# marco-conciatori-public/weed_instance_segmentation

Hardware: AMD Instinct MI355X
Metric: images/sec at 1024x1024 bs=8 per GPU (Mask2Former R50, 100 queries, fp32 forward-only) (higher is better)
Workload: dtype f32

## Files before the change

include/wm2f.h:

```cpp
#ifndef WM2F_H
#define WM2F_H

#include <stdint.h>

#ifdef __cplusplus
extern "C" {
#endif

#define WM2F_VERSION 100

#define WM2F_F32 0
#define WM2F_BF16 1
#define WM2F_I32 2
#define WM2F_U8 3
#define WM2F_U16 4
#define WM2F_I64 5

#define WM2F_OK 0
#define WM2F_EINVAL (-1)
#define WM2F_EUNSUPPORTED (-2)
#define WM2F_ELAUNCH (-3)

#define WM2F_MAX_LEVELS 8

// ... 128 lines not shown
                                 const void* pos, void* y, void* y_bf16, void* y_plus_pos, int yp_dtype, void* stats,
                                 int64_t rows, int C, int64_t pos_rows, float eps, float clamp, void* stream);
int wm2f_add_layernorm_train_bwd(const void* x, int x_dtype, const void* residual, const void* gamma, const void* stats,
                                 const void* grad_y, const void* grad_y_bf16, const void* grad_y_plus_pos, int gyp_dtype,
                                 void* grad_sum, void* grad_x, void* grad_gamma, void* grad_beta, void* workspace,
                                 int64_t rows, int C, void* stream);
int wm2f_token_linear_fwd(const void* x, const void* w, const void* bias, const void* residual, const void* ln_gamma,
                          const void* ln_beta, const void* pos, void* out, void* out_plus_pos, int64_t M, int K, int N, int relu,
                          int64_t pos_rows, float eps, int out_group, void* stream);

int wm2f_token_linear_split_weight(const void* w, void* w_split, int N, int K, void* stream);
int wm2f_token_linear_split_fwd(const void* x, const void* w_split, const void* bias, const void* residual, const void* ln_gamma,
                                const void* ln_beta, const void* pos, void* out, void* out_plus_pos, int64_t M, int K, int N,
                                int relu, int64_t pos_rows, float eps, int out_group, void* stream);

int wm2f_conv1x1_split_fwd(const void* x, const void* w_split, const void* bias, const void* residual, void* out, int B, int K,
                           int N, int Hi, int Wi, int stride, int relu, int config, void* stream);
int wm2f_conv1x1_split_config(int N, int P, int B, int n_cu);

int wm2f_conv3x3_split_fwd(const void* x, const void* w_split, const void* bias, void* out, int B, int Cin, int N, int Hi,
                           int Wi, int stride, int relu, int config, void* stream);
int wm2f_conv3x3_split_config(int N, int P, int B, int n_cu);

int wm2f_conv1x1_split_gn_fwd(const void* x, const void* w_split, const void* bias, void* out, void* stats_out, int G_out,
                              const void* norm_stats, const void* norm_gamma, const void* norm_beta, int norm_G, float norm_eps,
                              int norm_relu, int B, int K, int N, int Hi, int Wi, int stride, int config, void* stream);
int wm2f_conv3x3_split_stats_fwd(const void* x, const void* w_split, void* out, void* stats_out, int G_out, int B, int Cin,
                                 int N, int Hi, int Wi, int stride, int config, void* stream);
int wm2f_group_norm_act_apply(const void* x, const void* gamma, const void* beta, const void* up, void* y, const void* stats,
                              int B, int C, int G, int H, int W, int Hs, int Ws, float eps, int relu, void* stream);
int wm2f_group_norm_tokens_apply(const void* x, const void* bias, const void* gamma, const void* beta, void* tokens,
                                 const void* stats, int B, int C, int G, int HW, int S, int start, float eps, void* stream);

int wm2f_stem7x7_pool_fwd(const void* x, const void* w_split, const void* bias, void* out, int B, int Cin, int N, int Hi,
                          int Wi, int grid, void* stream);

int wm2f_token_linear_split_fwd_p(const void* x, const void* w_split, const void* bias, const void* residual,
                                  const void* ln_gamma, const void* ln_beta, const void* pos, void* out, void* out_plus_pos,
                                  int64_t M, int K, int N, int relu, int64_t pos_rows, float eps, int out_group, int pieces,
                                  void* stream);
int wm2f_conv1x1_split_fwd_p(const void* x, const void* w_split, const void* bias, const void* residual, void* out, int B, int K,
                             int N, int Hi, int Wi, int stride, int relu, int config, int pieces, void* stream);
int wm2f_conv1x1_split_gn_fwd_p(const void* x, const void* w_split, const void* bias, void* out, void* stats_out, int G_out,
                                const void* norm_stats, const void* norm_gamma, const void* norm_beta, int norm_G, float norm_eps,
                                int norm_relu, int B, int K, int N, int Hi, int Wi, int stride, int config, int pieces,
                                void* stream);
int wm2f_conv3x3_split_fwd_p(const void* x, const void* w_split, const void* bias, void* out, int B, int Cin, int N, int Hi,
                             int Wi, int stride, int relu, int config, int pieces, void* stream);
int wm2f_conv3x3_split_stats_fwd_p(const void* x, const void* w_split, void* out, void* stats_out, int G_out, int B, int Cin,
                                   int N, int Hi, int Wi, int stride, int config, int pieces, void* stream);
int wm2f_stem7x7_pool_fwd_p(const void* x, const void* w_split, const void* bias, void* out, int B, int Cin, int N, int Hi,
                            int Wi, int grid, int pieces, void* stream);

int64_t wm2f_token_wgrad_workspace(int64_t M, int N, int K);
int wm2f_token_wgrad_bf16(const void* dy, const void* x, void* dw, void* db, void* workspace, int64_t M, int N, int K,
// ... 229 lines not shown
```

weed_instance_segmentation_amd/_lib.py:

```python
from __future__ import annotations

import ctypes
import os
from ctypes import POINTER, c_char_p, c_float, c_int, c_int32, c_int64, c_void_p

HERE = os.path.dirname(os.path.abspath(__file__))
LIB_PATH = os.path.join(HERE, "libwm2f.so")
PROF_LIB_PATH = os.path.join(HERE, "libwm2f_prof.so")
if os.environ.get("WM2F_PROF_LIB"):
    PROF_LIB_PATH = os.environ["WM2F_PROF_LIB"]

WM2F_F32 = 0
WM2F_BF16 = 1
WM2F_I32 = 2
WM2F_U8 = 3
WM2F_U16 = 4
WM2F_I64 = 5
WM2F_CCL_VALUE, WM2F_CCL_BINARY, WM2F_CCL_RGB = 0, 1, 2
WM2F_CCL_MAX_COLORS = 16
WM2F_POLY_MAX_SIDE = 16384
WM2F_POLY_MAX_COORD = 1 << 24
WM2F_RLE_MAX_IDS = 1024
WM2F_AUG_MAX_VIRTUAL = 65536
WM2F_TILE_MAX_SIDE, WM2F_TILE_MAX_IDS, WM2F_TILE_MAX_TILES, WM2F_TILE_MAX_PAIRS = 16384, 256, 1024, 16384
# ... 65 lines not shown
    "wm2f_matcher_workspace": (c_int64, [_I, _I, _I, _I, _I]),
    "wm2f_matcher_cost": (c_int, [_P, _P, _P, _I, _HOST_I32, _P, _P, _P, _P, _I, _I, _I, _I, _I, _I, _I, _I, _I, _I,
                                  c_float, c_float, c_float, _P]),
    "wm2f_matcher_cost_levels": (c_int, [POINTER(c_void_p), _P, _P, _I, _HOST_I32, _P, _P, _P, _P, _I, _I, _I, _I, _I, _I, _I,
                                         _I, _I, _I, c_float, c_float, c_float, _P]),
    "wm2f_lsa_batched": (c_int, [_P, _P, _P, _P, _I, _I, _I, _I, _I, _P]),
    "wm2f_add_broadcast": (c_int, [_P, _P, _P, _I, c_int64, _P]),
    "wm2f_bias_act": (c_int, [_P, _P, _P, _P, _I, _I, _I, _I, _P]),
    "wm2f_add_layernorm": (c_int, [_P, _P, _P, _P, _P, _P, _P, c_int64, _I, c_int64, c_float, _P]),
    "wm2f_add_layernorm_train_workspace": (c_int64, [c_int64]),
    "wm2f_add_layernorm_train_fwd": (c_int, [_P, _I, _P, _P, _P, _P, _P, _P, _P, _I, _P, c_int64, _I, c_int64, c_float, c_float, _P]),
    "wm2f_add_layernorm_train_bwd": (c_int, [_P, _I, _P, _P, _P, _P, _P, _P, _I, _P, _P, _P, _P, _P, c_int64, _I, _P]),
    "wm2f_token_linear_fwd": (c_int, [_P, _P, _P, _P, _P, _P, _P, _P, _P, c_int64, _I, _I, _I, c_int64, c_float, _I, _P]),
    "wm2f_token_linear_split_weight": (c_int, [_P, _P, _I, _I, _P]),
    "wm2f_token_linear_split_fwd": (c_int, [_P, _P, _P, _P, _P, _P, _P, _P, _P, c_int64, _I, _I, _I, c_int64, c_float, _I, _P]),
    "wm2f_conv1x1_split_config": (c_int, [_I, _I, _I, _I]),
    "wm2f_conv1x1_split_fwd": (c_int, [_P, _P, _P, _P, _P, _I, _I, _I, _I, _I, _I, _I, _I, _P]),
    "wm2f_conv3x3_split_config": (c_int, [_I, _I, _I, _I]),
    "wm2f_conv3x3_split_fwd": (c_int, [_P, _P, _P, _P, _I, _I, _I, _I, _I, _I, _I, _I, _P]),
    "wm2f_conv1x1_split_gn_fwd": (c_int, [_P, _P, _P, _P, _P, _I, _P, _P, _P, _I, c_float, _I, _I, _I, _I, _I, _I, _I, _I, _P]),
    "wm2f_conv3x3_split_stats_fwd": (c_int, [_P, _P, _P, _P, _I, _I, _I, _I, _I, _I, _I, _I, _P]),
    "wm2f_group_norm_act_apply": (c_int, [_P, _P, _P, _P, _P, _P, _I, _I, _I, _I, _I, _I, _I, c_float, _I, _P]),
    "wm2f_group_norm_tokens_apply": (c_int, [_P, _P, _P, _P, _P, _P, _I, _I, _I, _I, _I, _I, c_float, _P]),
    "wm2f_stem7x7_pool_fwd":(c_int, [_P, _P, _P, _P, _I, _I, _I, _I, _I, _I, _P]),
    "wm2f_token_linear_split_fwd_p": (c_int, [_P, _P, _P, _P, _P, _P, _P, _P, _P, c_int64, _I, _I, _I, c_int64, c_float, _I, _I, _P]),
    "wm2f_conv1x1_split_fwd_p": (c_int, [_P, _P, _P, _P, _P, _I, _I, _I, _I, _I, _I, _I, _I, _I, _P]),
    "wm2f_conv1x1_split_gn_fwd_p": (c_int, [_P, _P, _P, _P, _P, _I, _P, _P, _P, _I, c_float, _I, _I, _I, _I, _I, _I, _I, _I, _I, _P]),
    "wm2f_conv3x3_split_fwd_p": (c_int, [_P, _P, _P, _P, _I, _I, _I, _I, _I, _I, _I, _I, _I, _P]),
    "wm2f_conv3x3_split_stats_fwd_p": (c_int, [_P, _P, _P, _P, _I, _I, _I, _I, _I, _I, _I, _I, _I, _P]),
    "wm2f_stem7x7_pool_fwd_p": (c_int, [_P, _P, _P, _P, _I, _I, _I, _I, _I, _I, _I, _P]),
    "wm2f_token_wgrad_workspace": (c_int64, [c_int64, _I, _I]),
    "wm2f_token_wgrad_bf16": (c_int, [_P, _P, _P, _P, _P, c_int64, _I, _I, _P]),
    "wm2f_token_wgrad_f32": (c_int, [_P, _P, _P, _P, _P, c_int64, _I, _I, _P]),
    "wm2f_tokens_to_nchw": (c_int, [_P, _P, _I, _I, _I, _I, _I, _P]),
    "wm2f_group_norm_tokens": (c_int, [_P, _P, _P, _P, _P, _P, _I, _I, _I, _I, _I, _I, c_float, _P]),
    "wm2f_resize_bilinear": (c_int, [_P, _P, _I, _I, _I, _I, _I, _P]),
    "wm2f_resize_pyramid": (c_int, [_P, _P, _P, _P, _I, _I, _I, _P]),
    "wm2f_bias_relu_maxpool": (c_int, [_P, _P, _P, _I, _I, _I, _I, _P]),
    "wm2f_group_norm_act": (c_int, [_P, _P, _P, _P, _P, _P, _I, _I, _I, _I, _I, _I, _I, c_float, _I, _P]),
    "wm2f_point_sample_fwd": (c_int, [_P, _I, _P, _P, _P, _I, _I, _I, _I, _P]),
# ... 112 lines not shown
```

weed_instance_segmentation_amd/csrc/token_gemm_split.hip:

```cpp
#include "common.h"

namespace wm2f {
namespace {

using f32x4 = __attribute__((ext_vector_type(4))) float;
using f32x8 = __attribute__((ext_vector_type(8))) float;
using u32x4 = __attribute__((ext_vector_type(4))) unsigned int;
using bf16x8 = __attribute__((ext_vector_type(8))) __bf16;
typedef __attribute__((address_space(3))) void* lds_ptr_t;

constexpr int kSgWaves = 8;
constexpr int kSgThreads = kSgWaves * 64;
constexpr int kSgCT = 2;
constexpr int kKStep = 32;
constexpr int kFrag = 1024;
constexpr unsigned kOob = 0x80000000u;
constexpr float kBf16Max = 3.38953139e38f;

template <int P = 3>
__device__ __forceinline__ void split3(const f32x8 x, bf16x8& h, bf16x8& m, bf16x8& l) {
  f32x8 xc;
#pragma unroll
  for (int i = 0; i < 8; ++i) xc[i] = __builtin_amdgcn_fmed3f(x[i], -kBf16Max, kBf16Max);
  if constexpr (P == 1) {
// ... 5 lines not shown
    const f32x8 r1 = x - __builtin_convertvector(h, f32x8);
    m = __builtin_convertvector(r1, bf16x8);
    if constexpr (P >= 3) {
      const f32x8 r2 = r1 - __builtin_convertvector(m, f32x8);
      l = __builtin_convertvector(r2, bf16x8);
    }
  }
}

__global__ __launch_bounds__(256) void split_weight_kernel(const float* __restrict__ w, bf16x8* __restrict__ ws, int N, int K) {
  const int kg_n = K / 8;
  const int i = blockIdx.x * blockDim.x + threadIdx.x;
  if (i >= N * kg_n) return;
  const int n = i / kg_n, kg = i - n * kg_n;
  const f32x4* src = reinterpret_cast<const f32x4*>(w + (int64_t)n * K + kg * 8);
  const f32x4 lo = src[0], hi = src[1];
  const f32x8 v = {lo[0], lo[1], lo[2], lo[3], hi[0], hi[1], hi[2], hi[3]};
  bf16x8 h, m, l;
  split3(v, h, m, l);
  const int ks = kg >> 2, g = kg & 3, rt = n >> 4, lane = (n & 15) + 16 * g;
  const int64_t base = ((int64_t)ks * (N / 16) + rt) * 3 * 64 + lane;
  ws[base] = h;
  ws[base + 64] = m;
  ws[base + 128] = l;
}

struct SgArgs {
  const float *x, *bias, *residual, *gamma, *beta, *pos;
  const void* ws;
  float *out, *out_pos;
// ... 265 lines not shown
          } else {
#pragma unroll
            for (int rt = 0; rt < NRT; ++rt)
              __builtin_amdgcn_raw_buffer_store_b128(__builtin_bit_cast(u32x4, acc[rt][c]), o_rs, row_o + (unsigned)((rt * 16 + 4 * g) * 4), 0, 0);
          }
        }
#pragma unroll
        for (int rt = 0; rt < NRT; ++rt) acc[rt][c] = (f32x4){0.f, 0.f, 0.f, 0.f};
      }
    }
    if (q + 1 < n_q && late) issue(q + 1);
    sg_barrier();
  }
}

using sg_kernel_t = void (*)(SgArgs);

template <bool PIPE, int ABL, int P = 3>
sg_kernel_t sg_pick(bool n288, int epi) {
  if (n288) return epi == 2 ? token_gemm_split_kernel<18, 2, PIPE, ABL, P> : (epi == 1 ? token_gemm_split_kernel<18, 1, true, ABL, P> : token_gemm_split_kernel<18, 0, true, ABL, P>);
  return epi == 2 ? token_gemm_split_kernel<16, 2, PIPE, ABL, P> : (epi == 1 ? token_gemm_split_kernel<16, 1, true, ABL, P> : token_gemm_split_kernel<16, 0, true, ABL, P>);
}

int device_cu_count(int* n_cu) {
  static int cached = 0;
  if (cached == 0) {
    int dev = 0;
    hipDeviceProp_t prop;
    if (hipGetDevice(&dev) != hipSuccess || hipGetDeviceProperties(&prop, dev) != hipSuccess) return -1;
    cached = prop.multiProcessorCount;
// ... 5 lines not shown
}
}

using namespace wm2f;

extern "C" int wm2f_token_linear_split_weight(const void* w, void* w_split, int N, int K, void* stream) {
  const char* who = "wm2f_token_linear_split_weight";
  WM2F_REQUIRE(w && w_split, "%s: null pointer", who);
  WM2F_REQUIRE(N > 0 && K > 0 && N % 16 == 0 && K % kKStep == 0, "%s: N = %d must be a multiple of 16 and K = %d of %d", who, N, K, kKStep);
  WM2F_REQUIRE((int64_t)N * K * 6 < (1ll << 31), "%s: the split weight must stay below 2 GiB", who);
  const int total = N * (K / 8);
  hipLaunchKernelGGL(split_weight_kernel, dim3((total + 255) / 256), dim3(256), 0, (hipStream_t)stream, (const float*)w,
                     (bf16x8*)w_split, N, K);
  WM2F_CHECK_LAUNCH(who);
  return WM2F_OK;
}

static int token_split_launch(const char* who, const void* x, const void* w_split, const void* bias, const void* residual,
                              const void* ln_gamma, const void* ln_beta, const void* pos, void* out, void* out_plus_pos,
                              int64_t M, int K, int N, int relu, int64_t pos_rows, float eps, int out_group, int pieces,
                              void* stream) {
  WM2F_REQUIRE(pieces >= 1 && pieces <= 3, "%s: pieces = %d (1, 2 and 3 are built)", who, pieces);
  WM2F_REQUIRE(x && w_split && bias && out, "%s: null pointer", who);
  WM2F_REQUIRE(M > 0 && K > 0 && N > 0, "%s: non-positive size", who);
  WM2F_REQUIRE(N == 256 || N == 288 || N == 512 || N == 768 || N == 1024,
               "%s: N = %d is not built (256, 288 and multiples of 256 up to 1024 are)", who, N);
  WM2F_REQUIRE(K % kKStep == 0, "%s: K = %d must be a multiple of %d", who, K, kKStep);
  WM2F_REQUIRE(M * (int64_t)K * 4 < (1ll << 31) && M * (int64_t)N * 4 < (1ll << 31), "%s: x / out must stay below 2 GiB (32-bit buffer offsets)", who);
  WM2F_REQUIRE((int64_t)N * K * 6 < (1ll << 31), "%s: the split weight must stay below 2 GiB", who);
  WM2F_REQUIRE(pos_rows * (int64_t)N * 4 < (1ll << 31), "%s: pos must stay below 2 GiB", who);
// ... 79 lines not shown
```

weed_instance_segmentation_amd/modeling.py:

```python
from __future__ import annotations

import json
import math
import os
from typing import Sequence

import numpy as np
import torch
import torch.nn.functional as F
from torch import nn

from . import ops
from .backbone_resnet import build_backbone
from .configuration import Mask2FormerConfig
from .loss import Mask2FormerLoss


class Mask2FormerForUniversalSegmentationOutput:

    _fields = ("loss", "class_queries_logits", "masks_queries_logits", "auxiliary_logits", "encoder_last_hidden_state",
               "pixel_decoder_last_hidden_state", "transformer_decoder_last_hidden_state", "encoder_hidden_states",
               "pixel_decoder_hidden_states", "transformer_decoder_hidden_states", "attentions")

    def __init__(self, **kw):
# ... 124 lines not shown
        self.self_attn_layer_norm = nn.LayerNorm(d)
        self.dropout = config.dropout
        self.fc1 = nn.Linear(d, config.encoder_feedforward_dim)
        self.fc2 = nn.Linear(config.encoder_feedforward_dim, d)
        self.final_layer_norm = nn.LayerNorm(d)

    def forward(self, hidden, pos, ref, level_hw, hp=None, emit_next=True):
        hidden_lp = None
        if isinstance(hp, tuple):
            hp, hidden_lp = hp
        if (not torch.is_grad_enabled() and self.dropout == 0.0 and hidden.shape[-1] == 256
                and hidden.dtype == torch.float32 and not torch.is_autocast_enabled("cuda")):
            B_, S_, C_ = hidden.shape
            ln1, ln2 = self.self_attn_layer_norm, self.final_layer_norm
            op = self.self_attn.output_proj
            if (ops.token_linear_applies(hidden, op.weight) and ops.token_linear_applies(hidden, self.fc1.weight)
                    and B_ * S_ * self.fc1.out_features * 4 < (1 << 31)):
                a = self.self_attn(hidden, pos, ref, level_hw, hp, project=False)
                hidden = ops.token_linear(a, op.weight, op.bias, residual=hidden, ln=(ln1.weight, ln1.bias, ln1.eps),
                                          w_split=ops.split_weight_cached(self, "output_proj", op.weight))
                f = ops.token_linear(hidden, self.fc1.weight, self.fc1.bias, relu=True,
                                     w_split=ops.split_weight_cached(self, "fc1", self.fc1.weight))
                return ops.token_linear(f, self.fc2.weight, self.fc2.bias, residual=hidden, ln=(ln2.weight, ln2.bias, ln2.eps),
                                        pos=pos, w_split=ops.split_weight_cached(self, "fc2", self.fc2.weight))
            a = self.self_attn(hidden, pos, ref, level_hw, hp)
            hidden = ops.add_layernorm(a, hidden, ln1.weight, ln1.bias, ln1.eps)
            f = torch._addmm_activation(self.fc1.bias, hidden.reshape(B_ * S_, C_), self.fc1.weight.t(), use_gelu=False)
            f = self.fc2(f).view(B_, S_, C_)
            return ops.add_layernorm(f, hidden, ln2.weight, ln2.bias, ln2.eps, pos=pos)
        amp = torch.is_autocast_enabled("cuda")
        bf16 = amp and torch.get_autocast_dtype("cuda") == torch.bfloat16
        if (torch.is_grad_enabled() and self.dropout == 0.0 and hidden.is_cuda and hidden.shape[-1] == 256
                and hidden.dtype == torch.float32 and (bf16 or not amp)):
            ln1, ln2 = self.self_attn_layer_norm, self.final_layer_norm
            a = self.self_attn(hidden, pos, ref, level_hw, hp, hidden_lp)
# ... 596 lines not shown
```

weed_instance_segmentation_amd/ops/__init__.py:

```python
from __future__ import annotations

import os as _os

K1_BWD_DETERMINISTIC: bool | None = None

CONV1X1_SPLIT = True

CONV3X3_SPLIT = True

CONV_GN_FUSED = True

SPLIT_PRECISION: str | None = _os.environ.get("WM2F_SPLIT_PRECISION") or "highest"

from .._lib import check
from ._core import KernelTimer, _p, _stream, set_kernel_timer
from .ccl import label_components, resize_nearest_tables
from .clean import labelmap_clean
from .copy_paste import copy_paste
from .fused import (add_broadcast, bias_act_, bias_relu_maxpool, group_norm_act_, group_norm_act_from_stats_, group_norm_tokens_,
                    group_norm_tokens_from_stats_, resize_bilinear, resize_pyramid, tokens_to_nchw)
from .gemm import (conv1x1, conv1x1_applies, conv1x1_gn, conv3x3, conv3x3_applies, conv3x3_stats, conv_group_stats_applies,
                   linear_tokens, split_weight, split_weight_3x3,
                   split_weight_cached, split_weight_stem, stem_conv_pool, stem_conv_pool_applies, stem_weight_columns,
                   stem_weight_matrix, token_linear, token_linear_applies, token_wgrad, token_wgrad_applies)
from .k1 import (k1_bwd_deterministic, k1_lane_order, k1_lane_rows, k1_lanes_applies, k1_rows_applies, ms_deform_attn,
                 ms_deform_attn_bwd, ms_deform_attn_fused, ms_deform_attn_fused_lanes, ms_deform_attn_fused_packed,
                 ms_deform_attn_rows, ms_deform_attn_variant)
from .k2 import masked_xattn, masked_xattn_bf16_applies
from .k3 import (attn_mask_build, mask_einsum, mask_einsum_attn_mask, mask_einsum_bf16, mask_einsum_bf16_bwd,
                 mask_einsum_bf16_bwd_applies, mask_einsum_bwd, mask_einsum_bwd_applies, nchw_to_pixel_major_bf16)
from .labelmaps import (coco_match, coco_match_min, labelmap_aim_points, labelmap_boundary, labelmap_distance,
                        labelmap_instance_stats, labelmap_pair_counts, labelmap_to_masks, mask_pair_counts, panoptic_match,
                        semantic_confusion_)
from .layernorm import add_layernorm, add_layernorm_train, add_layernorm_train_applies
from .loss import mask_loss_rows, point_sample, point_sample_levels, select_top_points
from .matcher import lsa_batched, matcher_cost
from .overlay import labelmap_overlay
from .polygons import fill_polygons
from .postprocess import (_GRID, instance_any, instance_maps, instance_scores, instance_segmentation, panoptic_probs,
# ... 10 lines not shown
```

weed_instance_segmentation_amd/ops/gemm.py:

```python
from __future__ import annotations

import weakref

import torch

from .. import ops as _flags
from .._lib import load
from ._core import _launch, _p, _req
from .fused import bias_act_, bias_relu_maxpool


_LEVEL_PIECES = {None: 3, "highest": 3, "high": 2, "medium": 1}


def _split_pieces():
    level = _flags.SPLIT_PRECISION
    if not (level is None or isinstance(level, str)) or level not in _LEVEL_PIECES:
        raise ValueError(f"ops.SPLIT_PRECISION = {level!r}: 'highest', 'high', 'medium' or None")
    pieces = _LEVEL_PIECES[level]
    return pieces, ("" if pieces == 3 else f"_p{pieces}")


def token_linear_applies(x: torch.Tensor, weight: torch.Tensor) -> bool:
    N, K = weight.shape
    M = x.numel() // max(K, 1)
    return (x.is_cuda and x.dtype == torch.float32 and weight.dtype == torch.float32 and N in (256, 288, 512, 768, 1024)
            and K % 32 == 0 and x.shape[-1] == K and M * K * 4 < (1 << 31) and M * N * 4 < (1 << 31)
            and N * K * 6 < (1 << 31))


def split_weight(weight: torch.Tensor) -> torch.Tensor:
    weight = _req(weight, "weight")
    N, K = weight.shape
    ws = torch.empty(N * K * 6, device=weight.device, dtype=torch.uint8)
    _launch("wm2f_token_linear_split_weight", weight, _p(weight), _p(ws), N, K)
    return ws


def split_weight_cached(owner, name: str, weight: torch.Tensor, base: torch.Tensor | None = None,
                        tap_major: bool = False) -> torch.Tensor:
    ident = weight if base is None else base
    c = owner.__dict__.setdefault("_wm2f_split", {})
    key = (ident._version, weight.data_ptr(), weight.device, tuple(weight.shape))
    hit = c.get(name)
    if hit is None or hit[0]() is not ident or hit[1] != key:
        if not tap_major:
            ws = split_weight(weight)
        else:
            ws = split_weight_stem(weight) if tuple(weight.shape[2:]) == (7, 7) else split_weight_3x3(weight)
        hit = (weakref.ref(ident), key, ws)
        c[name] = hit
    return hit[2]


def split_weight_3x3(weight: torch.Tensor) -> torch.Tensor:
    N = int(weight.shape[0])
    return split_weight(weight.permute(0, 2, 3, 1).reshape(N, -1).contiguous())


def token_linear(x: torch.Tensor, weight: torch.Tensor, bias: torch.Tensor, relu: bool = False, residual: torch.Tensor | None = None,
                 ln: tuple | None = None, pos: torch.Tensor | None = None, out_group: int = 0, split: bool = True,
                 w_split: torch.Tensor | None = None):
    x, weight, bias = _req(x, "x"), _req(weight, "weight"), _req(bias, "bias")
    N, K = weight.shape
    if x.shape[-1] != K or bias.shape != (N,):
        raise ValueError(f"token_linear: x {tuple(x.shape)} weight {tuple(weight.shape)} bias {tuple(bias.shape)}")
    M = x.numel() // K
# ... 20 lines not shown
    if split:
        if w_split is None:
            w_split = split_weight(weight)
        elif w_split.dtype != torch.uint8 or w_split.numel() != N * K * 6 or w_split.device != x.device:
            raise ValueError("token_linear: w_split is not split_weight(weight)")
        pieces, lvl = _split_pieces()
        _launch("wm2f_token_linear_split_fwd_p", x, _p(x), _p(w_split), _p(bias), _p(residual), _p(gamma), _p(beta), _p(pos),
                _p(out), _p(out_pos), M, K, N, 1 if relu else 0, pos_rows, eps, int(out_group), pieces,
                tag=tag + "_split" + lvl)
    else:
        _launch("wm2f_token_linear_fwd", x, _p(x), _p(weight), _p(bias), _p(residual), _p(gamma), _p(beta), _p(pos), _p(out),
                _p(out_pos), M, K, N, 1 if relu else 0, pos_rows, eps, int(out_group), tag=tag)
    return (out, out_pos) if pos is not None else out


def conv1x1_applies(x: torch.Tensor, weight: torch.Tensor, stride: int = 1) -> bool:
    if x.dim() != 4 or weight.dim() not in (2, 4) or (weight.dim() == 4 and weight.shape[2:] != (1, 1)):
        return False
    N, K = int(weight.shape[0]), int(weight.shape[1])
    _, C, H, W = x.shape
    Ho, Wo = (H - 1) // stride + 1, (W - 1) // stride + 1
    return (x.is_cuda and x.dtype == torch.float32 and weight.dtype == torch.float32 and C == K and K % 32 == 0
            and N % 64 == 0 and stride in (1, 2) and K * H * W * 4 < (1 << 31) and N * Ho * Wo * 4 < (1 << 31)
            and N * K * 6 < (1 << 31))


def conv1x1(x: torch.Tensor, weight: torch.Tensor, bias: torch.Tensor | None = None, residual: torch.Tensor | None = None,
            relu: bool = False, stride: int = 1, split: bool = True, w_split: torch.Tensor | None = None,
            config: int = -1) -> torch.Tensor:
    if residual is not None and (bias is None or not relu):
# ... 257 lines not shown
```

Measured before the change: 273.5.

## Fuse encoder feed-forward fc1+ReLU+fc2+residual+LayerNorm into one split-bf16 kernel

Adds a fused token FFN kernel that keeps each 16-token tile's hidden activations in registers. It streams fc1 and fc2 weight panels through LDS and applies bias, ReLU, residual, LayerNorm and the positional add in one pass. fc1 rows are pre-permuted so that the MFMA output fragments line up as the second GEMM's input, which removes the write and re-read of the large hidden tensor and one kernel launch per layer. In exchange the fc1 weight panels are streamed again for every tile, and each wave processes tiles serially with high register pressure.

```diff
diff --git a/include/wm2f.h b/include/wm2f.h
--- a/include/wm2f.h
+++ b/include/wm2f.h
@@ -166,6 +166,14 @@
                                 const void* ln_beta, const void* pos, void* out, void* out_plus_pos, int64_t M, int K, int N,
                                 int relu, int64_t pos_rows, float eps, int out_group, void* stream);
 
+#define WM2F_ROWS_NATURAL 0
+#define WM2F_ROWS_FFN 1
+int wm2f_token_linear_split_weight_rows(const void* w, void* w_split, int N, int K, int row_order, void* stream);
+int wm2f_token_ffn_row(int n);
+int wm2f_token_ffn_split_fwd(const void* x, const void* w1_split, const void* b1, const void* w2_split, const void* b2,
+                             const void* residual, const void* ln_gamma, const void* ln_beta, const void* pos, void* out,
+                             void* out_plus_pos, int64_t M, int K, int F, int N, int64_t pos_rows, float eps, void* stream);
+
 int wm2f_conv1x1_split_fwd(const void* x, const void* w_split, const void* bias, const void* residual, void* out, int B, int K,
                            int N, int Hi, int Wi, int stride, int relu, int config, void* stream);
 int wm2f_conv1x1_split_config(int N, int P, int B, int n_cu);
@@ -191,6 +199,10 @@
                                   const void* ln_gamma, const void* ln_beta, const void* pos, void* out, void* out_plus_pos,
                                   int64_t M, int K, int N, int relu, int64_t pos_rows, float eps, int out_group, int pieces,
                                   void* stream);
+int wm2f_token_ffn_split_fwd_p(const void* x, const void* w1_split, const void* b1, const void* w2_split, const void* b2,
+                               const void* residual, const void* ln_gamma, const void* ln_beta, const void* pos, void* out,
+                               void* out_plus_pos, int64_t M, int K, int F, int N, int64_t pos_rows, float eps, int pieces,
+                               void* stream);
 int wm2f_conv1x1_split_fwd_p(const void* x, const void* w_split, const void* bias, const void* residual, void* out, int B, int K,
                              int N, int Hi, int Wi, int stride, int relu, int config, int pieces, void* stream);
 int wm2f_conv1x1_split_gn_fwd_p(const void* x, const void* w_split, const void* bias, void* out, void* stats_out, int G_out,
diff --git a/weed_instance_segmentation_amd/_lib.py b/weed_instance_segmentation_amd/_lib.py
--- a/weed_instance_segmentation_amd/_lib.py
+++ b/weed_instance_segmentation_amd/_lib.py
@@ -103,6 +103,9 @@
     "wm2f_token_linear_fwd": (c_int, [_P, _P, _P, _P, _P, _P, _P, _P, _P, c_int64, _I, _I, _I, c_int64, c_float, _I, _P]),
     "wm2f_token_linear_split_weight": (c_int, [_P, _P, _I, _I, _P]),
     "wm2f_token_linear_split_fwd": (c_int, [_P, _P, _P, _P, _P, _P, _P, _P, _P, c_int64, _I, _I, _I, c_int64, c_float, _I, _P]),
+    "wm2f_token_linear_split_weight_rows": (c_int, [_P, _P, _I, _I, _I, _P]),
+    "wm2f_token_ffn_row": (c_int, [_I]),
+    "wm2f_token_ffn_split_fwd": (c_int, [_P, _P, _P, _P, _P, _P, _P, _P, _P, _P, _P, c_int64, _I, _I, _I, c_int64, c_float, _P]),
     "wm2f_conv1x1_split_config": (c_int, [_I, _I, _I, _I]),
     "wm2f_conv1x1_split_fwd": (c_int, [_P, _P, _P, _P, _P, _I, _I, _I, _I, _I, _I, _I, _I, _P]),
     "wm2f_conv3x3_split_config": (c_int, [_I, _I, _I, _I]),
@@ -113,6 +116,7 @@
     "wm2f_group_norm_tokens_apply": (c_int, [_P, _P, _P, _P, _P, _P, _I, _I, _I, _I, _I, _I, c_float, _P]),
     "wm2f_stem7x7_pool_fwd":(c_int, [_P, _P, _P, _P, _I, _I, _I, _I, _I, _I, _P]),
     "wm2f_token_linear_split_fwd_p": (c_int, [_P, _P, _P, _P, _P, _P, _P, _P, _P, c_int64, _I, _I, _I, c_int64, c_float, _I, _I, _P]),
+    "wm2f_token_ffn_split_fwd_p": (c_int, [_P, _P, _P, _P, _P, _P, _P, _P, _P, _P, _P, c_int64, _I, _I, _I, c_int64, c_float, _I, _P]),
     "wm2f_conv1x1_split_fwd_p": (c_int, [_P, _P, _P, _P, _P, _I, _I, _I, _I, _I, _I, _I, _I, _I, _P]),
     "wm2f_conv1x1_split_gn_fwd_p": (c_int, [_P, _P, _P, _P, _P, _I, _P, _P, _P, _I, c_float, _I, _I, _I, _I, _I, _I, _I, _I, _I, _P]),
     "wm2f_conv3x3_split_fwd_p": (c_int, [_P, _P, _P, _P, _I, _I, _I, _I, _I, _I, _I, _I, _I, _P]),
diff --git a/weed_instance_segmentation_amd/csrc/token_gemm_split.hip b/weed_instance_segmentation_amd/csrc/token_gemm_split.hip
--- a/weed_instance_segmentation_amd/csrc/token_gemm_split.hip
+++ b/weed_instance_segmentation_amd/csrc/token_gemm_split.hip
@@ -43,6 +43,27 @@
   if (i >= N * kg_n) return;
   const int n = i / kg_n, kg = i - n * kg_n;
   const f32x4* src = reinterpret_cast<const f32x4*>(w + (int64_t)n * K + kg * 8);
+  const f32x4 lo = src[0], hi = src[1];
+  const f32x8 v = {lo[0], lo[1], lo[2], lo[3], hi[0], hi[1], hi[2], hi[3]};
+  bf16x8 h, m, l;
+  split3(v, h, m, l);
+  const int ks = kg >> 2, g = kg & 3, rt = n >> 4, lane = (n & 15) + 16 * g;
+  const int64_t base = ((int64_t)ks * (N / 16) + rt) * 3 * 64 + lane;
+  ws[base] = h;
+  ws[base + 64] = m;
+  ws[base + 128] = l;
+}
+
+__host__ __device__ constexpr int ffn_row_of(int n) {
+  return (n & ~31) + 8 * ((n >> 2) & 3) + 4 * ((n >> 4) & 1) + (n & 3);
+}
+
+__global__ __launch_bounds__(256) void split_weight_rows_kernel(const float* __restrict__ w, bf16x8* __restrict__ ws, int N, int K) {
+  const int kg_n = K / 8;
+  const int i = blockIdx.x * blockDim.x + threadIdx.x;
+  if (i >= N * kg_n) return;
+  const int n = i / kg_n, kg = i - n * kg_n;
+  const f32x4* src = reinterpret_cast<const f32x4*>(w + (int64_t)ffn_row_of(n) * K + kg * 8);
   const f32x4 lo = src[0], hi = src[1];
   const f32x8 v = {lo[0], lo[1], lo[2], lo[3], hi[0], hi[1], hi[2], hi[3]};
   bf16x8 h, m, l;
@@ -338,6 +359,242 @@
   }
 }
 
+struct FfnArgs {
+  const float *x, *b1, *b2, *residual, *gamma, *beta, *pos;
+  const void *w1s, *w2s;
+  float *out, *out_pos;
+  int64_t M;
+  int F;
+  int64_t pos_rows;
+  float eps;
+  int tiles_total;
+};
+
+template <int ABL = 0, int P = 3>
+__global__ __launch_bounds__(kSgThreads) void token_ffn_split_kernel(FfnArgs a) {
+  constexpr int NRT = 16, D = 256, NKS = D / kKStep;
+  static_assert(P >= 1 && P <= 3, "one, two or three pieces");
+  constexpr int kPanelBytes = NRT * P * kFrag;
+  constexpr int kPieces = NRT * P;
+  extern __shared__ __attribute__((aligned(16))) unsigned char smem[];
+  const int tid = threadIdx.x, lane = tid & 63, wave = __builtin_amdgcn_readfirstlane(tid >> 6);
+  const int n_cu = gridDim.x, cu = blockIdx.x;
+  const int t0 = (int)(((int64_t)a.tiles_total * cu) / n_cu), t1 = (int)(((int64_t)a.tiles_total * (cu + 1)) / n_cu);
+  const int n_t = t1 - t0;
+  const int n_sl = a.F / D;
+  const int nrt1 = a.F / 16;
+  const int n_iter = (n_t + kSgWaves - 1) / kSgWaves;
+  float* vec = reinterpret_cast<float*>(smem + 2 * kPanelBytes);
+  for (int i = tid; i < a.F + 3 * D; i += kSgThreads) {
+    const int r = i - a.F;
+    vec[i] = r < 0 ? a.b1[i] : (r < D ? a.b2[r] : (r < 2 * D ? a.gamma[r - D] : a.beta[r - 2 * D]));
+  }
+  __syncthreads();
+  if (n_iter == 0) return;
+
+  const int base = n_t / kSgWaves, extra = n_t % kSgWaves;
+  const int w0 = t0 + wave * base + (wave < extra ? wave : extra);
+  const int w1 = w0 + base + (wave < extra ? 1 : 0);
+  const int g = lane >> 4, j = lane & 15;
+  const __amdgpu_buffer_rsrc_t w1_rs = __builtin_amdgcn_make_buffer_rsrc((void*)a.w1s, 0, a.F * D * 6, 0x00020000);
+  const __amdgpu_buffer_rsrc_t w2_rs = __builtin_amdgcn_make_buffer_rsrc((void*)a.w2s, 0, a.F * D * 6, 0x00020000);
+  const __amdgpu_buffer_rsrc_t x_rs = __builtin_amdgcn_make_buffer_rsrc((void*)a.x, 0, (int)(a.M * D * 4), 0x00020000);
+  const __amdgpu_buffer_rsrc_t o_rs = __builtin_amdgcn_make_buffer_rsrc((void*)a.out, 0, (int)(a.M * D * 4), 0x00020000);
+
+  auto issue_w = [&](const __amdgpu_buffer_rsrc_t rs, int src, int slot) {
+    unsigned char* dst = smem + slot * kPanelBytes;
+    for (int f = wave; f < kPieces; f += kSgWaves) {
+      const int fs = P == 3 ? f : (f / P) * 3 + f % P;
+      __builtin_amdgcn_raw_ptr_buffer_load_lds(rs, (lds_ptr_t)(dst + f * kFrag), 16, lane * 16, src + fs * kFrag, 0, 0);
+    }
+  };
+  auto w1_src = [&](int sl, int ks) { return (ks * nrt1 + sl * NRT) * 3 * kFrag; };
+  auto w2_src = [&](int sl, int i) { return (sl * NKS + i) * NRT * 3 * kFrag; };
+  f32x8 xr;
+  auto issue_x = [&](int tile, int ks) {
+    const int64_t t = (int64_t)tile * 16 + j;
+    const unsigned xo = (tile < w1 && t < a.M) ? (unsigned)((t * D + ks * kKStep + 8 * g) * 4) : kOob;
+    const f32x4 lo = __builtin_bit_cast(f32x4, __builtin_amdgcn_raw_buffer_load_b128(x_rs, xo, 0, 0));
+    const f32x4 hi = __builtin_bit_cast(f32x4, __builtin_amdgcn_raw_buffer_load_b128(x_rs, xo, 16, 0));
+    xr = (f32x8){lo[0], lo[1], lo[2], lo[3], hi[0], hi[1], hi[2], hi[3]};
+  };
+  auto k_step = [&](f32x4 (&acc)[NRT], int slot, const bf16x8 bh, const bf16x8 bm, const bf16x8 bl) {
+    const unsigned char* panel = smem + slot * kPanelBytes;
+    auto read_a = [&](bf16x8 (&dst)[3], int rt) {
+#pragma unroll
+      for (int p = 0; p < P; ++p) dst[p] = *reinterpret_cast<const bf16x8*>(panel + (rt * P + p) * kFrag + lane * 16);
+    };
+    bf16x8 av[2][3];
+    read_a(av[0], 0);
+#pragma unroll
+    for (int rt = 0; rt < NRT; ++rt) {
+      if (rt + 1 < NRT) read_a(av[(rt + 1) & 1], rt + 1);
+      __builtin_amdgcn_sched_barrier(0);
+      f32x4 c = acc[rt];
+      const bf16x8(&v)[3] = av[rt & 1];
+      if (ABL & kAblMfma) {
+        c[0] += __builtin_bit_cast(f32x4, v[0])[0] * __builtin_bit_cast(f32x4, bl)[0];
+        c[1] += __builtin_bit_cast(f32x4, v[1])[1] * __builtin_bit_cast(f32x4, bm)[1];
+        c[2] += __builtin_bit_cast(f32x4, v[2])[2] * __builtin_bit_cast(f32x4, bh)[2];
+      } else {
+        if constexpr (P == 3) {
+          c = __builtin_amdgcn_mfma_f32_16x16x32_bf16(v[1], bm, c, 0, 0, 0);
+          c = __builtin_amdgcn_mfma_f32_16x16x32_bf16(v[2], bh, c, 0, 0, 0);
+          c = __builtin_amdgcn_mfma_f32_16x16x32_bf16(v[0], bl, c, 0, 0, 0);
+        }
+        if constexpr (P >= 2) {
+          c = __builtin_amdgcn_mfma_f32_16x16x32_bf16(v[1], bh, c, 0, 0, 0);
+          c = __builtin_amdgcn_mfma_f32_16x16x32_bf16(v[0], bm, c, 0, 0, 0);
+        }
+        c = __builtin_amdgcn_mfma_f32_16x16x32_bf16(v[0], bh, c, 0, 0, 0);
+      }
+      acc[rt] = c;
+      __builtin_amdgcn_sched_barrier(0);
+    }
+  };
+
+  issue_w(w1_rs, w1_src(0, 0), 0);
+  issue_x(w0, 0);
+  sg_barrier();
+
+  f32x4 acc1[NRT], acc2[NRT];
+  for (int it = 0; it < n_iter; ++it) {
+    const int tile = w0 + it;
+    const bool live = tile < w1;
+#pragma unroll
+    for (int rt = 0; rt < NRT; ++rt) acc2[rt] = (f32x4){0.f, 0.f, 0.f, 0.f};
+
+    for (int sl = 0; sl < n_sl; ++sl) {
+      const bool more = sl + 1 < n_sl;
+#pragma unroll
+      for (int rt = 0; rt < NRT; ++rt) acc1[rt] = (f32x4){0.f, 0.f, 0.f, 0.f};
+#pragma unroll 1
+      for (int ks = 0; ks < NKS; ++ks) {
+        bf16x8 bh, bm, bl;
+        if (live) split3<P>(xr, bh, bm, bl);
+        const bool last = ks + 1 == NKS;
+        issue_w(last ? w2_rs : w1_rs, last ? w2_src(sl, 0) : w1_src(sl, ks + 1), (ks + 1) & 1);
+        issue_x(last && !more ? tile + 1 : tile, last ? 0 : ks + 1);
+        if (live) k_step(acc1, ks & 1, bh, bm, bl);
+        sg_barrier();
+      }
+      if (live) {
+#pragma unroll
+        for (int rt = 0; rt < NRT; ++rt) {
+          const f32x4 v = acc1[rt] + *reinterpret_cast<const f32x4*>(vec + sl * D + 32 * (rt >> 1) + 8 * g + 4 * (rt & 1));
+          f32x4 m = __builtin_elementwise_max(v, (f32x4){0.f, 0.f, 0.f, 0.f});
+#pragma unroll
+          for (int e = 0; e < 4; ++e) m[e] = v[e] != v[e] ? v[e] : m[e];
+          acc1[rt] = m;
+        }
+      }
+#pragma unroll
+      for (int i = 0; i < NKS; ++i) {
+        bf16x8 bh, bm, bl;
+        if (live) {
+          const f32x4 lo = acc1[2 * i], hi = acc1[2 * i + 1];
+          split3<P>((f32x8){lo[0], lo[1], lo[2], lo[3], hi[0], hi[1], hi[2], hi[3]}, bh, bm, bl);
+        }
+        if (i + 1 < NKS) {
+          issue_w(w2_rs, w2_src(sl, i + 1), (i + 1) & 1);
+        } else if (more) {
+          issue_w(w1_rs, w1_src(sl + 1, 0), 0);
+        }
+        if (live) k_step(acc2, i & 1, bh, bm, bl);
+        if (i + 1 < NKS || more) sg_barrier();
+      }
+    }
+
+    __builtin_amdgcn_sched_barrier(0);
+    if (live) {
+      const int64_t tk = (int64_t)tile * 16 + j;
+      const bool tok_ok = tk < a.M;
+      const unsigned row_g = tok_ok ? (unsigned)((tk * D + 4 * g) * 4) : kOob;
+      const bool st = !(ABL & kAblStores) || a.tiles_total < 0;
+      constexpr int kEB = 2;
+      const float* b2v = vec + a.F;
+#pragma unroll
+      for (int rt = 0; rt < NRT; ++rt) acc2[rt] = acc2[rt] + *reinterpret_cast<const f32x4*>(b2v + rt * 16 + 4 * g);
+      {
+        const __amdgpu_buffer_rsrc_t r_rs = __builtin_amdgcn_make_buffer_rsrc((void*)a.residual, 0, (int)(a.M * D * 4), 0x00020000);
+        f32x4 rv[2][kEB];
+#pragma unroll
+        for (int i = 0; i < kEB; ++i)
+          rv[0][i] = __builtin_bit_cast(f32x4, __builtin_amdgcn_raw_buffer_load_b128(r_rs, row_g, i * 64, 0));
+#pragma unroll
+        for (int h0 = 0; h0 < NRT; h0 += kEB) {
+          const int b = (h0 / kEB) & 1;
+          if (h0 + kEB < NRT) {
+#pragma unroll
+            for (int i = 0; i < kEB; ++i)
+              rv[b ^ 1][i] = __builtin_bit_cast(f32x4, __builtin_amdgcn_raw_buffer_load_b128(r_rs, row_g, (h0 + kEB + i) * 64, 0));
+          }
+#pragma unroll
+          for (int i = 0; i < kEB; ++i) acc2[h0 + i] += rv[b][i];
+          __builtin_amdgcn_sched_barrier(0);
+        }
+      }
+      float s1 = 0.f, s2 = 0.f;
+#pragma unroll
+      for (int rt = 0; rt < NRT; ++rt) {
+        const f32x4 v = acc2[rt];
+        s1 += (v[0] + v[1]) + (v[2] + v[3]);
+        s2 += (v[0] * v[0] + v[1] * v[1]) + (v[2] * v[2] + v[3] * v[3]);
+      }
+      s1 += __shfl_xor(s1, 16, 64);
+      s1 += __shfl_xor(s1, 32, 64);
+      s2 += __shfl_xor(s2, 16, 64);
+      s2 += __shfl_xor(s2, 32, 64);
+      const float inv_n = 1.f / (float)D;
+      const float mean = s1 * inv_n;
+      float var = s2 * inv_n - mean * mean;
+      var = var < 0.f ? 0.f : var;
+      const float rstd = rsqrtf(var + a.eps);
+#pragma unroll
+      for (int rt = 0; rt < NRT; ++rt) {
+        const int f0 = rt * 16 + 4 * g;
+        const f32x4 gm = *reinterpret_cast<const f32x4*>(b2v + D + f0), bt = *reinterpret_cast<const f32x4*>(b2v + 2 * D + f0);
+        acc2[rt] = (acc2[rt] - mean) * rstd * gm + bt;
+      }
+      if (!a.out_pos) {
+        if (st) {
+#pragma unroll
+          for (int rt = 0; rt < NRT; ++rt)
+            __builtin_amdgcn_raw_buffer_store_b128(__builtin_bit_cast(u32x4, acc2[rt]), o_rs, row_g, rt * 64, 0);
+        }
+      } else {
+        const __amdgpu_buffer_rsrc_t p_rs = __builtin_amdgcn_make_buffer_rsrc((void*)a.pos, 0, (int)(a.pos_rows * D * 4), 0x00020000);
+        const __amdgpu_buffer_rsrc_t q_rs = __builtin_amdgcn_make_buffer_rsrc((void*)a.out_pos, 0, (int)(a.M * D * 4), 0x00020000);
+        const unsigned prow = tok_ok ? (unsigned)(((tk % a.pos_rows) * D + 4 * g) * 4) : kOob;
+        f32x4 pv[2][kEB];
+#pragma unroll
+        for (int i = 0; i < kEB; ++i)
+          pv[0][i] = __builtin_bit_cast(f32x4, __builtin_amdgcn_raw_buffer_load_b128(p_rs, prow, i * 64, 0));
+#pragma unroll
+        for (int h0 = 0; h0 < NRT; h0 += kEB) {
+          const int b = (h0 / kEB) & 1;
+          if (h0 + kEB < NRT) {
+#pragma unroll
+            for (int i = 0; i < kEB; ++i)
+              pv[b ^ 1][i] = __builtin_bit_cast(f32x4, __builtin_amdgcn_raw_buffer_load_b128(p_rs, prow, (h0 + kEB + i) * 64, 0));
+          }
+          if (st) {
+#pragma unroll
+            for (int i = 0; i < kEB; ++i)
+              __builtin_amdgcn_raw_buffer_store_b128(__builtin_bit_cast(u32x4, acc2[h0 + i]), o_rs, row_g, (h0 + i) * 64, 0);
+#pragma unroll
+            for (int i = 0; i < kEB; ++i)
+              __builtin_amdgcn_raw_buffer_store_b128(__builtin_bit_cast(u32x4, acc2[h0 + i] + pv[b][i]), q_rs, row_g, (h0 + i) * 64, 0);
+          }
+          __builtin_amdgcn_sched_barrier(0);
+        }
+      }
+    }
+    if (it + 1 < n_iter) issue_w(w1_rs, w1_src(0, 0), 0);
+    sg_barrier();
+  }
+}
+
 using sg_kernel_t = void (*)(SgArgs);
 
 template <bool PIPE, int ABL, int P = 3>
@@ -373,6 +630,97 @@
                      (bf16x8*)w_split, N, K);
   WM2F_CHECK_LAUNCH(who);
   return WM2F_OK;
+}
+
+extern "C" int wm2f_token_linear_split_weight_rows(const void* w, void* w_split, int N, int K, int row_order, void* stream) {
+  const char* who = "wm2f_token_linear_split_weight_rows";
+  WM2F_REQUIRE(row_order == WM2F_ROWS_NATURAL || row_order == WM2F_ROWS_FFN, "%s: row_order = %d (0: natural, 1: the fused feed-forward's)", who, row_order);
+  if (row_order == WM2F_ROWS_NATURAL) return wm2f_token_linear_split_weight(w, w_split, N, K, stream);
+  WM2F_REQUIRE(w && w_split, "%s: null pointer", who);
+  WM2F_REQUIRE(N > 0 && K > 0 && N % 32 == 0 && K % kKStep == 0, "%s: N = %d and K = %d must be multiples of %d", who, N, K, kKStep);
+  WM2F_REQUIRE((int64_t)N * K * 6 < (1ll << 31), "%s: the split weight must stay below 2 GiB", who);
+  const int total = N * (K / 8);
+  hipLaunchKernelGGL(split_weight_rows_kernel, dim3((total + 255) / 256), dim3(256), 0, (hipStream_t)stream, (const float*)w,
+                     (bf16x8*)w_split, N, K);
+  WM2F_CHECK_LAUNCH(who);
+  return WM2F_OK;
+}
+
+extern "C" int wm2f_token_ffn_row(int n) { return n >= 0 ? ffn_row_of(n) : -1; }
+
+static int token_ffn_launch(const char* who, const void* x, const void* w1_split, const void* b1, const void* w2_split,
+                            const void* b2, const void* residual, const void* ln_gamma, const void* ln_beta, const void* pos,
+                            void* out, void* out_plus_pos, int64_t M, int K, int F, int N, int64_t pos_rows, float eps,
+                            int pieces, void* stream) {
+  WM2F_REQUIRE(pieces >= 1 && pieces <= 3, "%s: pieces = %d (1, 2 and 3 are built)", who, pieces);
+  WM2F_REQUIRE(x && w1_split && b1 && w2_split && b2 && out, "%s: null pointer", who);
+  WM2F_REQUIRE(residual && ln_gamma && ln_beta, "%s: the residual and the LayerNorm (gamma and beta) are part of the kernel", who);
+  WM2F_REQUIRE(M > 0, "%s: non-positive size", who);
+  WM2F_REQUIRE(K == 256 && N == 256, "%s: K = %d, N = %d (256 and 256 are built)", who, K, N);
+  WM2F_REQUIRE(F == 256 || F == 512 || F == 768 || F == 1024, "%s: F = %d is not built (256, 512, 768 and 1024 are)", who, F);
+  WM2F_REQUIRE(M * (int64_t)256 * 4 < (1ll << 31), "%s: x / out must stay below 2 GiB (32-bit buffer offsets)", who);
+  WM2F_REQUIRE((pos == nullptr) == (out_plus_pos == nullptr), "%s: pos and out_plus_pos come together", who);
+  WM2F_REQUIRE(!pos || (pos_rows > 0 && pos_rows * (int64_t)256 * 4 < (1ll << 31)), "%s: pos needs pos_rows >= 1 and must stay below 2 GiB", who);
+  int n_cu = 0;
+  if (device_cu_count(&n_cu) != 0) {
+    set_error("%s: cannot query the device", who);
+    return WM2F_ELAUNCH;
+  }
+  FfnArgs a;
+  a.x = (const float*)x;
+  a.w1s = w1_split;
+  a.w2s = w2_split;
+  a.b1 = (const float*)b1;
+  a.b2 = (const float*)b2;
+  a.residual = (const float*)residual;
+  a.gamma = (const float*)ln_gamma;
+  a.beta = (const float*)ln_beta;
+  a.pos = (const float*)pos;
+  a.out = (float*)out;
+  a.out_pos = (float*)out_plus_pos;
+  a.M = M;
+  a.F = F;
+  a.pos_rows = pos_rows;
+  a.eps = eps;
+  a.tiles_total = (int)ceil_div64(M, 16);
+  int grid = n_cu;
+  if (grid > a.tiles_total) grid = a.tiles_total;
+  const size_t lds = (size_t)2 * 16 * pieces * kFrag + (size_t)(F + 3 * 256) * sizeof(float);
+  void (*kfn)(FfnArgs) = pieces == 3 ? token_ffn_split_kernel<0> : (pieces == 2 ? token_ffn_split_kernel<0, 2> : token_ffn_split_kernel<0, 1>);
+#ifdef WM2F_PROFILING
+  {
+    const char* ea = getenv("WM2F_FFN_ABL");
+    const int abl = ea ? atoi(ea) : 0;
+    WM2F_REQUIRE(abl == 0 || abl == 1 || abl == 4, "%s: WM2F_FFN_ABL = %d is not built (1 and 4 are)", who, abl);
+    WM2F_REQUIRE(pieces == 3 || abl == 0, "%s: WM2F_FFN_ABL is built for three pieces", who);
+    if (abl == 1) kfn = token_ffn_split_kernel<kAblStores>;
+    if (abl == 4) kfn = token_ffn_split_kernel<kAblMfma>;
+  }
+#endif
+  hipError_t e = hipFuncSetAttribute((const void*)kfn, hipFuncAttributeMaxDynamicSharedMemorySize, (int)lds);
+  if (e != hipSuccess) {
+    set_error("%s: cannot raise dynamic LDS to %zu: %s", who, lds, hipGetErrorString(e));
+    return WM2F_ELAUNCH;
+  }
+  hipLaunchKernelGGL(kfn, dim3(grid), dim3(kSgThreads), lds, (hipStream_t)stream, a);
+  WM2F_CHECK_LAUNCH(who);
+  return WM2F_OK;
+}
+
+extern "C" int wm2f_token_ffn_split_fwd(const void* x, const void* w1_split, const void* b1, const void* w2_split, const void* b2,
+                                        const void* residual, const void* ln_gamma, const void* ln_beta, const void* pos,
+                                        void* out, void* out_plus_pos, int64_t M, int K, int F, int N, int64_t pos_rows,
+                                        float eps, void* stream) {
+  return token_ffn_launch("wm2f_token_ffn_split_fwd", x, w1_split, b1, w2_split, b2, residual, ln_gamma, ln_beta, pos, out,
+                          out_plus_pos, M, K, F, N, pos_rows, eps, 3, stream);
+}
+
+extern "C" int wm2f_token_ffn_split_fwd_p(const void* x, const void* w1_split, const void* b1, const void* w2_split,
+                                          const void* b2, const void* residual, const void* ln_gamma, const void* ln_beta,
+                                          const void* pos, void* out, void* out_plus_pos, int64_t M, int K, int F, int N,
+                                          int64_t pos_rows, float eps, int pieces, void* stream) {
+  return token_ffn_launch("wm2f_token_ffn_split_fwd_p", x, w1_split, b1, w2_split, b2, residual, ln_gamma, ln_beta, pos, out,
+                          out_plus_pos, M, K, F, N, pos_rows, eps, pieces, stream);
 }
 
 static int token_split_launch(const char* who, const void* x, const void* w_split, const void* bias, const void* residual,
diff --git a/weed_instance_segmentation_amd/modeling.py b/weed_instance_segmentation_amd/modeling.py
--- a/weed_instance_segmentation_amd/modeling.py
+++ b/weed_instance_segmentation_amd/modeling.py
@@ -162,11 +162,17 @@
             B_, S_, C_ = hidden.shape
             ln1, ln2 = self.self_attn_layer_norm, self.final_layer_norm
             op = self.self_attn.output_proj
+            fused = ops.TOKEN_FFN_FUSED and ops.token_ffn_applies(hidden, self.fc1.weight, self.fc2.weight)
             if (ops.token_linear_applies(hidden, op.weight) and ops.token_linear_applies(hidden, self.fc1.weight)
-                    and B_ * S_ * self.fc1.out_features * 4 < (1 << 31)):
+                    and (fused or B_ * S_ * self.fc1.out_features * 4 < (1 << 31))):
                 a = self.self_attn(hidden, pos, ref, level_hw, hp, project=False)
                 hidden = ops.token_linear(a, op.weight, op.bias, residual=hidden, ln=(ln1.weight, ln1.bias, ln1.eps),
                                           w_split=ops.split_weight_cached(self, "output_proj", op.weight))
+                if fused:
+                    return ops.token_ffn(hidden, self.fc1.weight, self.fc1.bias, self.fc2.weight, self.fc2.bias, hidden,
+                                         (ln2.weight, ln2.bias, ln2.eps), pos=pos,
+                                         w1_split=ops.split_weight_rows_cached(self, "fc1_ffn", self.fc1.weight),
+                                         w2_split=ops.split_weight_cached(self, "fc2", self.fc2.weight))
                 f = ops.token_linear(hidden, self.fc1.weight, self.fc1.bias, relu=True,
                                      w_split=ops.split_weight_cached(self, "fc1", self.fc1.weight))
                 return ops.token_linear(f, self.fc2.weight, self.fc2.bias, residual=hidden, ln=(ln2.weight, ln2.bias, ln2.eps),
diff --git a/weed_instance_segmentation_amd/ops/__init__.py b/weed_instance_segmentation_amd/ops/__init__.py
--- a/weed_instance_segmentation_amd/ops/__init__.py
+++ b/weed_instance_segmentation_amd/ops/__init__.py
@@ -10,6 +10,8 @@
 
 CONV_GN_FUSED = True
 
+TOKEN_FFN_FUSED = True
+
 SPLIT_PRECISION: str | None = _os.environ.get("WM2F_SPLIT_PRECISION") or "highest"
 
 from .._lib import check
@@ -20,9 +22,10 @@
 from .fused import (add_broadcast, bias_act_, bias_relu_maxpool, group_norm_act_, group_norm_act_from_stats_, group_norm_tokens_,
                     group_norm_tokens_from_stats_, resize_bilinear, resize_pyramid, tokens_to_nchw)
 from .gemm import (conv1x1, conv1x1_applies, conv1x1_gn, conv3x3, conv3x3_applies, conv3x3_stats, conv_group_stats_applies,
-                   linear_tokens, split_weight, split_weight_3x3,
-                   split_weight_cached, split_weight_stem, stem_conv_pool, stem_conv_pool_applies, stem_weight_columns,
-                   stem_weight_matrix, token_linear, token_linear_applies, token_wgrad, token_wgrad_applies)
+                   ROWS_FFN, ROWS_NATURAL, ffn_row_order, linear_tokens, split_weight, split_weight_3x3,
+                   split_weight_cached, split_weight_rows, split_weight_rows_cached, split_weight_stem, stem_conv_pool,
+                   stem_conv_pool_applies, stem_weight_columns, stem_weight_matrix, token_ffn, token_ffn_applies,
+                   token_linear, token_linear_applies, token_wgrad, token_wgrad_applies)
 from .k1 import (k1_bwd_deterministic, k1_lane_order, k1_lane_rows, k1_lanes_applies, k1_rows_applies, ms_deform_attn,
                  ms_deform_attn_bwd, ms_deform_attn_fused, ms_deform_attn_fused_lanes, ms_deform_attn_fused_packed,
                  ms_deform_attn_rows, ms_deform_attn_variant)
diff --git a/weed_instance_segmentation_amd/ops/gemm.py b/weed_instance_segmentation_amd/ops/gemm.py
--- a/weed_instance_segmentation_amd/ops/gemm.py
+++ b/weed_instance_segmentation_amd/ops/gemm.py
@@ -37,20 +37,43 @@
     return ws
 
 
-def split_weight_cached(owner, name: str, weight: torch.Tensor, base: torch.Tensor | None = None,
-                        tap_major: bool = False) -> torch.Tensor:
-    ident = weight if base is None else base
+ROWS_NATURAL, ROWS_FFN = 0, 1
+
+
+def ffn_row_order(n_rows: int) -> torch.Tensor:
+    lib = load()
+    return torch.tensor([lib.wm2f_token_ffn_row(n) for n in range(n_rows)], dtype=torch.long)
+
+
+def split_weight_rows(weight: torch.Tensor, row_order: int = ROWS_FFN) -> torch.Tensor:
+    weight = _req(weight, "weight")
+    N, K = weight.shape
+    ws = torch.empty(N * K * 6, device=weight.device, dtype=torch.uint8)
+    _launch("wm2f_token_linear_split_weight_rows", weight, _p(weight), _p(ws), N, K, int(row_order))
+    return ws
+
+
+def _split_cached(owner, name: str, weight: torch.Tensor, ident: torch.Tensor, make) -> torch.Tensor:
     c = owner.__dict__.setdefault("_wm2f_split", {})
     key = (ident._version, weight.data_ptr(), weight.device, tuple(weight.shape))
     hit = c.get(name)
     if hit is None or hit[0]() is not ident or hit[1] != key:
-        if not tap_major:
-            ws = split_weight(weight)
-        else:
-            ws = split_weight_stem(weight) if tuple(weight.shape[2:]) == (7, 7) else split_weight_3x3(weight)
-        hit = (weakref.ref(ident), key, ws)
+        hit = (weakref.ref(ident), key, make(weight))
         c[name] = hit
     return hit[2]
+
+
+def split_weight_cached(owner, name: str, weight: torch.Tensor, base: torch.Tensor | None = None,
+                        tap_major: bool = False) -> torch.Tensor:
+    if not tap_major:
+        make = split_weight
+    else:
+        make = split_weight_stem if tuple(weight.shape[2:]) == (7, 7) else split_weight_3x3
+    return _split_cached(owner, name, weight, weight if base is None else base, make)
+
+
+def split_weight_rows_cached(owner, name: str, weight: torch.Tensor, row_order: int = ROWS_FFN) -> torch.Tensor:
+    return _split_cached(owner, name, weight, weight, lambda w: split_weight_rows(w, row_order))
 
 
 def split_weight_3x3(weight: torch.Tensor) -> torch.Tensor:
@@ -101,6 +124,54 @@
     return (out, out_pos) if pos is not None else out
 
 
+def token_ffn_applies(x: torch.Tensor, w1: torch.Tensor, w2: torch.Tensor) -> bool:
+    if w1.dim() != 2 or w2.dim() != 2:
+        return False
+    F_, K = w1.shape
+    N = w2.shape[0]
+    M = x.numel() // max(K, 1)
+    return (x.is_cuda and x.dtype == torch.float32 and w1.dtype == torch.float32 and w2.dtype == torch.float32
+            and K == 256 and N == 256 and w2.shape[1] == F_ and F_ in (256, 512, 768, 1024) and x.shape[-1] == K
+            and M * 256 * 4 < (1 << 31))
+
+
+def token_ffn(x: torch.Tensor, w1: torch.Tensor, b1: torch.Tensor, w2: torch.Tensor, b2: torch.Tensor, residual: torch.Tensor,
+              ln: tuple, pos: torch.Tensor | None = None, w1_split: torch.Tensor | None = None,
+              w2_split: torch.Tensor | None = None):
+    x, w1, b1, w2, b2 = _req(x, "x"), _req(w1, "w1"), _req(b1, "b1"), _req(w2, "w2"), _req(b2, "b2")
+    F_, K = w1.shape
+    N = w2.shape[0]
+    if x.shape[-1] != K or b1.shape != (F_,) or w2.shape != (N, F_) or b2.shape != (N,):
+        raise ValueError(f"token_ffn: x {tuple(x.shape)} w1 {tuple(w1.shape)} b1 {tuple(b1.shape)} w2 {tuple(w2.shape)} "
+                         f"b2 {tuple(b2.shape)}")
+    if residual is None or ln is None:
+        raise ValueError("token_ffn: the residual and the LayerNorm are part of the kernel")
+    M = x.numel() // K
+    residual = _req(residual, "residual")
+    if residual.numel() != M * N:
+        raise ValueError("token_ffn: residual shape")
+    gamma, beta, eps = _req(ln[0], "gamma"), _req(ln[1], "beta"), float(ln[2])
+    out = torch.empty(*x.shape[:-1], N, device=x.device, dtype=torch.float32)
+    out_pos, pos_rows = None, 0
+    if pos is not None:
+        pos = _req(pos, "pos")
+        pos_rows = pos.numel() // N
+        if M % pos_rows:
+            raise ValueError("token_ffn: pos rows do not divide the token count")
+        out_pos = torch.empty_like(out)
+    for ws, what in ((w1_split, "w1_split is not split_weight_rows(w1, ROWS_FFN)"), (w2_split, "w2_split is not split_weight(w2)")):
+        if ws is not None and (ws.dtype != torch.uint8 or ws.numel() != F_ * K * 6 or ws.device != x.device):
+            raise ValueError("token_ffn: " + what)
+    if w1_split is None:
+        w1_split = split_weight_rows(w1, ROWS_FFN)
+    if w2_split is None:
+        w2_split = split_weight(w2)
+    pieces, lvl = _split_pieces()
+    _launch("wm2f_token_ffn_split_fwd_p", x, _p(x), _p(w1_split), _p(b1), _p(w2_split), _p(b2), _p(residual), _p(gamma), _p(beta),
+            _p(pos), _p(out), _p(out_pos), M, K, F_, N, pos_rows, eps, pieces, tag=f"token_ffn_K{K}_F{F_}_split" + lvl)
+    return (out, out_pos) if pos is not None else out
+
+
 def conv1x1_applies(x: torch.Tensor, weight: torch.Tensor, stride: int = 1) -> bool:
     if x.dim() != 4 or weight.dim() not in (2, 4) or (weight.dim() == 4 and weight.shape[2:] != (1, 1)):
         return False
```

Result: faster. 276.9, median of 6 (+1.2%).
